# mastbaum/sxmc

Measured on AMD Instinct MI355X. Metric: NLL evals/sec (10^8 samples, 3 obs, 12 signals) + experiments/sec at 1/2/4/8 GPUs, higher is better.
Workload: dtype f64 exact; f32-on-u16-codes filter decides the unambiguous samples

## Files before the change

### sxmc_amd/csrc/nll_device.h

```cpp
#pragma once

#include "sxmc_device.h"

#pragma clang fp contract(off)

namespace sxdev {

constexpr int kWave = 64;

struct Philox4 {
  unsigned x, y, z, w;
};

__device__ __forceinline__ Philox4 philox4x32_10(unsigned long long counter_lo,
                                                 unsigned long long counter_hi,
                                                 unsigned long long key) {
  unsigned c0 = (unsigned)counter_lo, c1 = (unsigned)(counter_lo >> 32);
  unsigned c2 = (unsigned)counter_hi, c3 = (unsigned)(counter_hi >> 32);
  unsigned k0 = (unsigned)key, k1 = (unsigned)(key >> 32);
#pragma unroll
  for (int r = 0; r < 10; r++) {
    const unsigned hi0 = __umulhi(0xD2511F53u, c0), lo0 = 0xD2511F53u * c0;
    const unsigned hi1 = __umulhi(0xCD9E8D57u, c2), lo1 = 0xCD9E8D57u * c2;
    const unsigned n0 = hi1 ^ c1 ^ k0, n1 = lo1, n2 = hi0 ^ c3 ^ k1, n3 = lo0;
    c0 = n0; c1 = n1; c2 = n2; c3 = n3;
    k0 += 0x9E3779B9u;
    k1 += 0xBB67AE85u;
  }
  return Philox4{c0, c1, c2, c3};
}

__device__ __forceinline__ Philox4 rng_next(sxmc_rng_state* st) {
  const Philox4 r = philox4x32_10(st->offset, st->subsequence, st->seed);
  st->offset += 1;
  return r;
}

__device__ __forceinline__ double rng_uniform(sxmc_rng_state* st) {
  const Philox4 r = rng_next(st);
  return ((double)r.x + 1.0) * 2.3283064365386963e-10;
}

__device__ __forceinline__ double rng_normal(sxmc_rng_state* st) {
  const Philox4 r = rng_next(st);
  const double u1 = ((double)r.x + 1.0) * 2.3283064365386963e-10;
  const double u2 = (double)r.y * 2.3283064365386963e-10;
  return sqrt(-2.0 * log(u1)) * cos(6.283185307179586 * u2);
}

__device__ __forceinline__ void pick_new_vector_device(int n, sxmc_rng_state* rng,
                                                       const float* jump_width,
                                                       const double* current_vector,
                                                       double* proposed_vector) {
  const int offset = blockIdx.x * blockDim.x + threadIdx.x;
  const int stride = gridDim.x * blockDim.x;
  for (int i = offset; i < n; i += stride) {
    if (jump_width[i] > 0) {
      const double u = rng_normal(&rng[i]);
      proposed_vector[i] = current_vector[i] + jump_width[i] * u;
    } else {
      proposed_vector[i] = current_vector[i];
    }
  }
}

__device__ __forceinline__ void jump_decider_device(sxmc_rng_state* rng, double* nll_current,
                                                    const double* nll_proposed, double* v_current,
                                                    const double* v_proposed, unsigned nparameters,
                                                    int* accepted, int* counter, float* jump_buffer,
                                                    bool debug_mode) {
  const double u = rng_uniform(&rng[0]);
  const double np = nll_proposed[0];
  const double nc = nll_current[0];
  if (debug_mode || (np < nc || u <= exp(nc - np))) {
    nll_current[0] = np;
    for (unsigned i = 0; i < nparameters; i++) v_current[i] = v_proposed[i];
    accepted[0] += 1;
  }
  const int count = counter[0];
  for (unsigned i = 0; i < nparameters; i++) {
    jump_buffer[count * (nparameters + 1) + i] = (float)v_current[i];
  }
  jump_buffer[count * (nparameters + 1) + nparameters] = (float)nll_current[0];
  counter[0] = count + 1;
}

__device__ __forceinline__ void nll_total_device(size_t nparameters, size_t nsignals, size_t nsources,
                                                 const double* pars, const double* means,
                                                 const double* sigmas, const double* events_total,
                                                 const double* nexpected, const unsigned* n_mc,
                                                 const short* source_id, const unsigned* norms,
                                                 double* nll) {
  double sum = -events_total[0];
  if (isnan(sum)) {
    nll[0] = 1e18;
    return;
  }
  for (unsigned i = 0; i < nsignals; i++) {
    const short sid = source_id[i];
    sum += pars[sid] * nexpected[i] * norms[i] / n_mc[i];
  }
  for (unsigned i = 0; i < nparameters; i++) {
    if (i < nsources && pars[i] < 0) {
      nll[0] = 1e18;
      return;
    }
    if (sigmas[i] > 0) {
      const double x = (pars[i] - means[i]) / sigmas[i];
      sum += 0.5 * x * x;
    }
  }
  nll[0] = sum;
}

template <int BD = 0>
__device__ __forceinline__ double block_sum(size_t n, const double* sums, double* s_wave ) {
  const unsigned bdim = BD > 0 ? (unsigned)BD : blockDim.x;
  double t = 0.0;
  size_t i = threadIdx.x;
  const size_t bd = bdim;
  for (; i + 15 * bd < n; i += 16 * bd) {
    double v[16];
#pragma unroll
    for (int k = 0; k < 16; k++) v[k] = sums[i + (size_t)k * bd];
#pragma unroll
    for (int k = 0; k < 16; k++) t += v[k];
  }
  for (; i < n; i += bd) t += sums[i];
  const int wave = threadIdx.x / kWave;
  const int lane = threadIdx.x & (kWave - 1);
  const int live = min(kWave, (int)bdim - wave * kWave);
#pragma unroll
  for (int off = kWave / 2; off > 0; off >>= 1) {
    const double o = __shfl_down(t, off, kWave);
    t += (lane + off < live) ? o : 0.0;
  }
  const int nwaves = ((int)bdim + kWave - 1) / kWave;
  if ((threadIdx.x & (kWave - 1)) == 0) s_wave[wave] = t;
  __syncthreads();
  if (threadIdx.x == 0) {
    double tot = 0.0;
    for (int w = 0; w < nwaves; w++) tot += s_wave[w];
    s_wave[16] = tot;
  }
  __syncthreads();
  return s_wave[16];
}

constexpr int kStage = 256;

template <int BD = 0, typename Wait>
__device__ __forceinline__ bool finish_step_device_w(size_t npartial_sums, const double* sums, size_t nsignals,
                                                     size_t nsources, const double* means, const double* sigmas,
                                                     sxmc_rng_state* rng, double* nll_current,
                                                     double* nll_proposed, double* v_current, double* v_proposed,
                                                     int* accepted, int* counter, float* jump_buffer,
                                                     int nparameters, const float* jump_width,
                                                     const double* nexpected, const unsigned* n_mc,
                                                     const short* source_id, const unsigned* norms,
                                                     bool debug_mode, Wait&& wait) {
  __shared__ double s_wave[17];
  __shared__ double s_vprop[kStage], s_vcur[kStage], s_pen[kStage], s_z[kStage], s_term[kStage];
  __shared__ float s_jw[kStage];
  __shared__ unsigned char s_flag[kStage];
  __shared__ int s_accept, s_count;
  __shared__ double s_nllcur, s_u;

  const unsigned bdim = BD > 0 ? (unsigned)BD : blockDim.x;
  const bool staged = nparameters <= kStage && nsignals <= (size_t)kStage;
  if (!staged) {
    wait();
    double total_sum = block_sum<BD>(npartial_sums, sums, s_wave);
    if (threadIdx.x == 0) {
      nll_total_device(nparameters, nsignals, nsources, v_proposed, means, sigmas, &total_sum, nexpected, n_mc,
                       source_id, norms, nll_proposed);
      jump_decider_device(rng, nll_current, nll_proposed, v_current, v_proposed, nparameters, accepted, counter,
                          jump_buffer, debug_mode);
    }
    __threadfence_block();
    __syncthreads();
    pick_new_vector_device(nparameters, rng, jump_width, v_current, v_proposed);
    __syncthreads();
    return nll_current[0] == nll_proposed[0];
  }

  double nc = 0.0;
  int count = 0;
  if (threadIdx.x == 0) {
    nc = nll_current[0];
    count = counter[0];
  }
  for (int i = threadIdx.x; i < nparameters; i += (int)bdim) {
    const double p = v_proposed[i], mean = means[i], sigma = sigmas[i];
    const float jw = jump_width[i];
    s_vprop[i] = p;
    s_vcur[i] = v_current[i];
    s_jw[i] = jw;
    unsigned char flag = 0;
    double pen = 0.0;
    if (sigma > 0) {
      const double x = (p - mean) / sigma;
      pen = 0.5 * x * x;
      flag |= 1;
    }
    if ((size_t)i < nsources && p < 0) flag |= 2;
    s_pen[i] = pen;
    s_flag[i] = flag;
    if (i == 0 || jw > 0) {
      sxmc_rng_state st = rng[i];
      if (i == 0) s_u = rng_uniform(&st);
      s_z[i] = (jw > 0) ? rng_normal(&st) : 0.0;
      rng[i].offset = st.offset;
    }
  }
  for (int j = threadIdx.x; j < (int)nsignals; j += (int)bdim) {
    s_term[j] = v_proposed[source_id[j]] * nexpected[j] * norms[j] / n_mc[j];
  }
  wait();
  const double total_sum = block_sum<BD>(npartial_sums, sums, s_wave);

  if (threadIdx.x == 0) {
    double sum = -total_sum;
    bool bad = isnan(sum);
    if (!bad) {
      for (unsigned j = 0; j < nsignals; j++) sum += s_term[j];
      for (int i = 0; i < nparameters; i++) {
        if (s_flag[i] & 2) {
          bad = true;
          break;
        }
        if (s_flag[i] & 1) sum += s_pen[i];
      }
    }
    const double np = bad ? 1e18 : sum;
    nll_proposed[0] = np;
    const bool accept = debug_mode || (np < nc || s_u <= exp(nc - np));
    if (accept) {
      nll_current[0] = np;
      accepted[0] += 1;
    }
    counter[0] = count + 1;
    s_accept = accept ? 1 : 0;
    s_count = count;
    s_nllcur = accept ? np : nc;
  }
  __syncthreads();

  const bool accept = s_accept != 0;
  const size_t row = (size_t)s_count * (size_t)(nparameters + 1);
  for (int i = threadIdx.x; i < nparameters; i += (int)bdim) {
    const double cur = accept ? s_vprop[i] : s_vcur[i];
    if (accept) v_current[i] = cur;
    jump_buffer[row + i] = (float)cur;
    v_proposed[i] = (s_jw[i] > 0) ? cur + s_jw[i] * s_z[i] : cur;
  }
  if (threadIdx.x == 0) jump_buffer[row + nparameters] = (float)s_nllcur;
  return accept;
}

__device__ __forceinline__ bool finish_step_device(size_t npartial_sums, const double* sums, size_t nsignals,
                                                   size_t nsources, const double* means, const double* sigmas,
                                                   sxmc_rng_state* rng, double* nll_current,
                                                   double* nll_proposed, double* v_current, double* v_proposed,
                                                   int* accepted, int* counter, float* jump_buffer,
                                                   int nparameters, const float* jump_width,
                                                   const double* nexpected, const unsigned* n_mc,
                                                   const short* source_id, const unsigned* norms,
                                                   bool debug_mode) {
  return finish_step_device_w<0>(npartial_sums, sums, nsignals, nsources, means, sigmas, rng, nll_current, nll_proposed,
                              v_current, v_proposed, accepted, counter, jump_buffer, nparameters, jump_width, nexpected,
                              n_mc, source_id, norms, debug_mode, [] {});
}

__device__ __forceinline__ void peek_next_proposal_device(int nparameters, const sxmc_rng_state* rng,
                                                          const float* jump_width, const double* v_current,
                                                          double* out) {
  for (int i = threadIdx.x; i < nparameters; i += blockDim.x) {
    const float jw = jump_width[i];
    double v = v_current[i];
    if (jw > 0) {
      sxmc_rng_state st = rng[i];
      if (i == 0) (void)rng_uniform(&st);
      v = v + jw * rng_normal(&st);
    }
    out[i] = v;
  }
}

}
```

### sxmc_amd/csrc/pdfz_kernels.hip

```cpp
#include <hip/hip_runtime.h>
#include <hip/hip_ext.h>

#include <algorithm>
#include <cstring>
#include <vector>

#include "nll_device.h"

#include "fill_kernels.inc.h"

#pragma clang fp contract(off)

namespace {

using namespace sxfill;


__global__ __launch_bounds__(256) void zero_kernel(const SxSignalDesc* __restrict__ descs, unsigned* ticket) {
  const SxSignalDesc& d = descs[blockIdx.y];
  unsigned* bins = d.bins;
  const unsigned n = (unsigned)d.total_nbins;
  const unsigned n4 = n >> 2;
  uint4* b4 = reinterpret_cast<uint4*>(bins);
  const unsigned stride = gridDim.x * blockDim.x;
// ... 147 lines not shown
};
struct MembersFromTable {
  static constexpr bool kTable = true;
  const SxSignalDesc* __restrict__ descs;
  const SxStepEndTable& t;
};

template <int BD = 0, typename Members, typename Ready>
__device__ __forceinline__ double eval_nll_block_part(const Members& mem, int nsig,
                                                      unsigned long long npoints, const unsigned* __restrict__ weight,
                                                      const double* __restrict__ pars,
                                                      const double* __restrict__ nexpected,
                                                      const unsigned* __restrict__ n_mc,
                                                      const short* __restrict__ source_id,
                                                      const unsigned* __restrict__ norms, double* sh,
                                                      unsigned block_index, unsigned nblocks, Ready&& ready) {
  constexpr bool kTable = Members::kTable;
  double* s_wave = sh;
  EvalMember* s_mem = reinterpret_cast<EvalMember*>(sh + 16);
  const unsigned bdim = BD > 0 ? (unsigned)BD : blockDim.x;

  constexpr int U = 16;
  static_assert(!kTable || U == SXMC_STEP_END_MEMBERS, "the table holds one pass of members");
  int rb[U];
  unsigned long long i = (unsigned long long)block_index * bdim + threadIdx.x;
  auto load_read_bins = [&](unsigned long long ev, int j0) {
    const unsigned long long evc = ev < npoints ? ev : npoints - 1;
    gptr<const int> table[U];
#pragma unroll
    for (int u = 0; u < U; u++) {
      if constexpr (kTable) table[u] = to_global(mem.t.read_bins[u]);
      else table[u] = to_global(mem.descs[min(j0 + u, nsig - 1)].read_bins);
    }
#pragma unroll
    for (int u = 0; u < U; u++) rb[u] = table[u][evc];
#pragma unroll
    for (int u = 0; u < U; u++) rb[u] = (j0 + u < nsig && ev < npoints) ? rb[u] : -2;
  };
  auto bins_of = [&](int j0, int u) {
    if constexpr (kTable) return to_global(mem.t.bins[u]);
    else return to_global(s_mem[j0 + u].bins);
  };
  if (npoints == 0 || nsig <= 0) {
    ready();
    return 0.0;
  }
  load_read_bins(i, 0);
  unsigned wfirst = weight ? to_global(weight)[i < npoints ? i : npoints - 1] : 1u;
  unsigned count[U];

  auto stage = [&](int j, const SxSignalDesc& d, unsigned normv, double volume, unsigned nj, unsigned nmc, double par,
                   double nexp) {
    s_mem[j].read_bins = d.read_bins;
    s_mem[j].bins = d.bins;
    s_mem[j].out = d.pdf_out;
    s_mem[j].stride = d.pdf_stride;
    s_mem[j].bin_norm = (double)normv * volume;
    const float eff = (float)(1.0 * nj / nmc);
    s_mem[j].coef = par * nexp * eff;
  };
  if constexpr (kTable) {
    const int j = min((int)threadIdx.x, nsig - 1);
    const SxSignalDesc& d = mem.descs[j];
    const unsigned* normp = d.norm;
    const double volume = d.bin_volume;
    const short sid = source_id[j];
    const unsigned nmc = n_mc[j];
    const double nexp = nexpected[j];
    ready();
    const unsigned nj = norms[j];
    const unsigned normv = *to_global(normp);
    const double par = pars[sid];
#pragma unroll
    for (int u = 0; u < U; u++) count[u] = bins_of(0, u)[rb[u] >= 0 ? rb[u] : 0];
#pragma unroll
    for (int u = 0; u < U; u++) count[u] = (rb[u] >= 0) ? count[u] : 0u;
    stage(j, d, normv, volume, nj, nmc, par, nexp);
  } else {
    ready();
    for (int j = threadIdx.x; j < nsig; j += (int)bdim) {
      const SxSignalDesc& d = mem.descs[j];
      stage(j, d, *to_global((const unsigned*)d.norm), d.bin_volume, norms[j], n_mc[j], pars[source_id[j]], nexpected[j]);
    }
  }
#if SXMC_WG_STAMPS
  if (kTable && BD == 0) {
    asm volatile("s_waitcnt vmcnt(0)" ::: "memory");
    SX_WG_STAMP(1);
  }
#endif
  __syncthreads();

  double sum = 0.0;
  bool requested = true;
  const unsigned long long step = (unsigned long long)nblocks * bdim;
  for (; i < npoints; i += step) {
    double s = 0.0;
    const unsigned wrow = requested ? wfirst : (weight ? to_global(weight)[i] : 1u);
    for (int j0 = 0; j0 < nsig; j0 += U) {
      const bool gathered = kTable && requested;
      if (!requested) load_read_bins(i, j0);
      requested = false;
      if (!gathered) {
#pragma unroll
        for (int u = 0; u < U; u++) count[u] = (rb[u] >= 0) ? bins_of(j0, u)[rb[u]] : 0u;
      }
#if SXMC_WG_STAMPS
      if (!kTable && BD == 0 && i < bdim * nblocks) {
        asm volatile("s_waitcnt vmcnt(0)" ::: "memory");
        SX_WG_STAMP(1);
      }
#endif
#pragma unroll
      for (int u = 0; u < U; u++) {
        if (j0 + u < nsig) {
          float v;
          if (rb[u] == -2) v = 0.0f;
          else if (rb[u] < 0) v = __int_as_float(0x7fc00000);
          else v = (float)((double)count[u] / s_mem[j0 + u].bin_norm);
          if (s_mem[j0 + u].out) to_global(s_mem[j0 + u].out)[s_mem[j0 + u].stride * (long)i] = v;
          s = s + s_mem[j0 + u].coef * (double)(!isnan(v) ? v : 0.0f);
        }
      }
    }
    if (s > 0) sum += weight ? (double)wrow * log(s) : log(s);
  }

#pragma unroll
  for (int off = kWave / 2; off > 0; off >>= 1) sum += __shfl_down(sum, off, kWave);
  const int wave = threadIdx.x / kWave;
  if ((threadIdx.x & (kWave - 1)) == 0) s_wave[wave] = sum;
  __syncthreads();
  double t = 0.0;
  if (threadIdx.x == 0) {
    for (int w = 0; w < (int)(bdim / kWave); w++) t += s_wave[w];
  }
  return t;
}

template <int BD = 0, typename Ready>
__device__ __forceinline__ double eval_nll_block_part(const SxSignalDesc* __restrict__ descs, int nsig,
                                                      unsigned long long npoints, const unsigned* __restrict__ weight,
                                                      const double* __restrict__ pars,
                                                      const double* __restrict__ nexpected,
                                                      const unsigned* __restrict__ n_mc,
                                                      const short* __restrict__ source_id,
                                                      const unsigned* __restrict__ norms, double* sh,
                                                      unsigned block_index, unsigned nblocks, Ready&& ready) {
  return eval_nll_block_part<BD>(MembersFromDescs{descs}, nsig, npoints, weight, pars, nexpected, n_mc, source_id, norms,
                                 sh, block_index, nblocks, ready);
}

template <int BD = 0>
__device__ __forceinline__ double eval_nll_block_part(const SxSignalDesc* __restrict__ descs, int nsig,
                                                      unsigned long long npoints, const unsigned* __restrict__ weight,
                                                      const double* __restrict__ pars,
                                                      const double* __restrict__ nexpected,
                                                      const unsigned* __restrict__ n_mc,
                                                      const short* __restrict__ source_id,
                                                      const unsigned* __restrict__ norms, double* sh,
                                                      unsigned block_index, unsigned nblocks) {
  return eval_nll_block_part<BD>(descs, nsig, npoints, weight, pars, nexpected, n_mc, source_id, norms, sh, block_index,
                                 nblocks, [] {});
}

__device__ __forceinline__ double eval_nll_block(const SxSignalDesc* __restrict__ descs, int nsig,
                                                 unsigned long long npoints, const unsigned* __restrict__ weight,
                                                 const double* __restrict__ pars,
                                                 const double* __restrict__ nexpected,
                                                 const unsigned* __restrict__ n_mc,
                                                 const short* __restrict__ source_id,
                                                 const unsigned* __restrict__ norms, double* sh) {
  return eval_nll_block_part(descs, nsig, npoints, weight, pars, nexpected, n_mc, source_id, norms, sh, blockIdx.x,
                             gridDim.x);
}

__global__ __launch_bounds__(256) void eval_nll_kernel(const SxSignalDesc* __restrict__ descs, int nsig,
                                                       unsigned long long npoints,
                                                       const unsigned* __restrict__ weight,
                                                       const double* __restrict__ pars,
                                                       const double* __restrict__ nexpected,
                                                       const unsigned* __restrict__ n_mc,
                                                       const short* __restrict__ source_id,
                                                       const unsigned* __restrict__ norms,
                                                       double* __restrict__ sums) {
  extern __shared__ double sh[];
  const double t = eval_nll_block(descs, nsig, npoints, weight, pars, nexpected, n_mc, source_id, norms, sh);
  if (threadIdx.x == 0 && !isnan(t)) sums[blockIdx.x] = t;
}

__global__ __launch_bounds__(256) void eval_nll_finish_kernel(const SxSignalDesc* __restrict__ descs, int nsig,
                                                              unsigned long long npoints,
                                                              const unsigned* __restrict__ weight, double* sums,
                                                              unsigned* ticket, SxStepArgs a) {
  extern __shared__ double sh[];
  const double t =
      eval_nll_block(descs, nsig, npoints, weight, a.v_proposed, a.nexpected, a.n_mc, a.source_id, a.norms, sh);
  int* s_last = reinterpret_cast<int*>(sh + 15);
  if (threadIdx.x == 0) {
    sums[blockIdx.x] = isnan(t) ? 0.0 : t;
    asm volatile("s_waitcnt vmcnt(0)" ::: "memory");
    __builtin_amdgcn_fence(__ATOMIC_RELEASE, "agent");
    asm volatile("s_waitcnt vmcnt(0)" ::: "memory");
    const unsigned arrived = __hip_atomic_fetch_add(ticket, 1u, __ATOMIC_RELAXED, __HIP_MEMORY_SCOPE_AGENT);
    const int last = arrived == gridDim.x - 1u;
    if (last) {
      __builtin_amdgcn_fence(__ATOMIC_ACQUIRE, "agent");
      asm volatile("s_waitcnt vmcnt(0)" ::: "memory");
    }
    *s_last = last;
  }
  __syncthreads();
  if (!*s_last) return;
  __syncthreads();
  sxdev::finish_step_device(gridDim.x, sums, a.nsignals, a.nsources, a.means, a.sigmas, a.rng, a.nll_current,
                            a.nll_proposed, a.v_current, a.v_proposed, a.accepted, a.counter, a.jump_buffer,
                            a.nparameters, a.jump_width, a.nexpected, a.n_mc, a.source_id, a.norms,
                            a.debug_mode != 0);
}

__global__ __launch_bounds__(256) void eval_nll2_kernel(const SxSignalDesc* __restrict__ descs_a,
                                                        const SxSignalDesc* __restrict__ descs_b, int nsig,
                                                        unsigned long long npoints,
                                                        const unsigned* __restrict__ weight_a,
                                                        const unsigned* __restrict__ weight_b,
                                                        const double* __restrict__ pars_a,
                                                        const double* __restrict__ pars_b,
                                                        const double* __restrict__ nexpected,
                                                        const unsigned* __restrict__ n_mc,
                                                        const short* __restrict__ source_id,
                                                        const unsigned* __restrict__ norms_a,
                                                        const unsigned* __restrict__ norms_b,
                                                        double* __restrict__ sums_a, double* __restrict__ sums_b,
                                                        unsigned half) {
  extern __shared__ double sh[];
  const bool second = blockIdx.x >= half;
  const double t = eval_nll_block_part(second ? descs_b : descs_a, nsig, npoints, second ? weight_b : weight_a,
                                       second ? pars_b : pars_a, nexpected, n_mc, source_id,
                                       second ? norms_b : norms_a, sh, second ? blockIdx.x - half : blockIdx.x, half);
  if (threadIdx.x == 0 && !isnan(t)) (second ? sums_b : sums_a)[second ? blockIdx.x - half : blockIdx.x] = t;
}

__global__ __launch_bounds__(256) void finish2_zero_kernel(const SxSignalDesc* __restrict__ descs_a,
                                                           const SxSignalDesc* __restrict__ descs_b, int nsig,
                                                           unsigned zblocks, size_t npartial, const double* sums_a,
                                                           const double* sums_b, const unsigned* norms_b, double* v_b,
                                                           const int* cap, SxStepArgs a) {
  if (blockIdx.x == 0) {
    __shared__ int s_before;
    if (threadIdx.x == 0) s_before = a.counter[0];
    __syncthreads();
    const int limit = cap ? cap[0] : 0x7FFFFFFF;
    if (s_before < limit) {
      const bool accepted =
          sxdev::finish_step_device(npartial, sums_a, a.nsignals, a.nsources, a.means, a.sigmas, a.rng, a.nll_current,
                                    a.nll_proposed, a.v_current, a.v_proposed, a.accepted, a.counter, a.jump_buffer,
                                    a.nparameters, a.jump_width, a.nexpected, a.n_mc, a.source_id, a.norms,
                                    a.debug_mode != 0);
      __syncthreads();
      if (!accepted && s_before + 1 < limit) {
        sxdev::finish_step_device(npartial, sums_b, a.nsignals, a.nsources, a.means, a.sigmas, a.rng, a.nll_current,
                                  a.nll_proposed, a.v_current, a.v_proposed, a.accepted, a.counter, a.jump_buffer,
                                  a.nparameters, a.jump_width, a.nexpected, a.n_mc, a.source_id, norms_b,
                                  a.debug_mode != 0);
        __syncthreads();
      }
      sxdev::peek_next_proposal_device(a.nparameters, a.rng, a.jump_width, a.v_current, v_b);
    }
    __syncthreads();
    for (int j = threadIdx.x; j < nsig; j += blockDim.x) {
      *descs_a[j].norm = 0u;
      *descs_b[j].norm = 0u;
    }
    return;
  }
  const unsigned b = blockIdx.x - 1u;
  const unsigned which = b / (zblocks * (unsigned)nsig);
  const unsigned bb = b - which * zblocks * (unsigned)nsig;
  const SxSignalDesc& d = (which ? descs_b : descs_a)[bb / zblocks];
  const unsigned chunk = bb % zblocks;
  unsigned* bins = d.bins;
  const unsigned n = (unsigned)d.total_nbins;
  const unsigned n4 = n >> 2;
  uint4* b4 = reinterpret_cast<uint4*>(bins);
  const unsigned stride = zblocks * blockDim.x;
  for (unsigned i = chunk * blockDim.x + threadIdx.x; i < n4; i += stride) b4[i] = make_uint4(0u, 0u, 0u, 0u);
  if (chunk == 0 && threadIdx.x < (n & 3u)) bins[(n4 << 2) + threadIdx.x] = 0u;
}

__global__ void peek_next_proposal_kernel(int nparameters, const sxmc_rng_state* rng, const float* jump_width,
                                          const double* v_current, double* out) {
  sxdev::peek_next_proposal_device(nparameters, rng, jump_width, v_current, out);
}

__global__ __launch_bounds__(1024) void tail_step_kernel(const SxSignalDesc* __restrict__ descs, int nsig,
                                                         unsigned long long npoints,
                                                         const unsigned* __restrict__ weight, SxStepArgs a) {
  extern __shared__ double sh[];
  __shared__ double s_total;
  const double t =
      eval_nll_block(descs, nsig, npoints, weight, a.v_proposed, a.nexpected, a.n_mc, a.source_id, a.norms, sh);
  if (threadIdx.x == 0) s_total = isnan(t) ? 0.0 : t;
  __syncthreads();
  sxdev::finish_step_device(1, &s_total, a.nsignals, a.nsources, a.means, a.sigmas, a.rng, a.nll_current,
                            a.nll_proposed, a.v_current, a.v_proposed, a.accepted, a.counter, a.jump_buffer,
                            a.nparameters, a.jump_width, a.nexpected, a.n_mc, a.source_id, a.norms,
                            a.debug_mode != 0);
  for (int j = 0; j < nsig; j++) {
    const SxSignalDesc& d = descs[j];
    const unsigned n = (unsigned)d.total_nbins, n4 = n >> 2;
    uint4* b4 = reinterpret_cast<uint4*>(d.bins);
    for (unsigned i = threadIdx.x; i < n4; i += blockDim.x) b4[i] = make_uint4(0u, 0u, 0u, 0u);
    if (threadIdx.x < (n & 3u)) d.bins[(n4 << 2) + threadIdx.x] = 0u;
    if (threadIdx.x == 0) *d.norm = 0u;
  }
}

__global__ __launch_bounds__(256) void finish_zero_kernel(const SxSignalDesc* __restrict__ descs, int nsig,
                                                          unsigned zblocks, size_t npartial, const double* sums,
                                                          unsigned* ticket, SxStepArgs a) {
  if (blockIdx.x == 0) {
    sxdev::finish_step_device(npartial, sums, a.nsignals, a.nsources, a.means, a.sigmas, a.rng, a.nll_current,
                              a.nll_proposed, a.v_current, a.v_proposed, a.accepted, a.counter, a.jump_buffer,
                              a.nparameters, a.jump_width, a.nexpected, a.n_mc, a.source_id, a.norms,
                              a.debug_mode != 0);
    __syncthreads();
    for (int j = threadIdx.x; j < nsig; j += blockDim.x) *descs[j].norm = 0u;
    if (threadIdx.x == 0 && ticket) *ticket = 0u;
    return;
  }
  const unsigned b = blockIdx.x - 1u;
  const SxSignalDesc& d = descs[b / zblocks];
  const unsigned chunk = b % zblocks;
  unsigned* bins = d.bins;
  const unsigned n = (unsigned)d.total_nbins;
  const unsigned n4 = n >> 2;
  uint4* b4 = reinterpret_cast<uint4*>(bins);
  const unsigned stride = zblocks * blockDim.x;
  for (unsigned i = chunk * blockDim.x + threadIdx.x; i < n4; i += stride) b4[i] = make_uint4(0u, 0u, 0u, 0u);
  if (chunk == 0 && threadIdx.x < (n & 3u)) bins[(n4 << 2) + threadIdx.x] = 0u;
}

constexpr unsigned kEndSpinLimit = 200000u;
constexpr unsigned long long kSlotEmpty = 0x7FF8DEADBEEF0001ull, kSlotNaN = 0x7FF8DEADBEEF0002ull;

template <int BD, typename Members, typename Ready>
__device__ __forceinline__ void step_end_role(unsigned role, unsigned W, const Members& lookup,
                                              const SxSignalDesc* __restrict__ hist_descs, int nsig,
                                              unsigned long long npoints, const unsigned* __restrict__ weight,
                                              unsigned long long* slots, double* last_good, unsigned* sync,
                                              unsigned nvb, unsigned zblocks, const SxStepArgs& a, double* sh,
                                              Ready&& ready) {
  const unsigned bdim = BD > 0 ? (unsigned)BD : blockDim.x;
  unsigned* const timeouts = sync + 6;
  if (role == W) {
    ready();
    __shared__ double s_part[128];
    sxdev::finish_step_device_w<BD>(nvb, s_part, a.nsignals, a.nsources, a.means, a.sigmas, a.rng, a.nll_current,
                                    a.nll_proposed, a.v_current, a.v_proposed, a.accepted, a.counter, a.jump_buffer,
                                    a.nparameters, a.jump_width, a.nexpected, a.n_mc, a.source_id, a.norms,
                                    a.debug_mode != 0, [&] {
                                      const unsigned i = threadIdx.x;
                                      if (i < nvb) {
                                        unsigned long long v = kSlotEmpty;
                                        unsigned it = 0;
                                        for (; it < kEndSpinLimit; it++) {
                                          v = __hip_atomic_load(slots + i, __ATOMIC_RELAXED, __HIP_MEMORY_SCOPE_AGENT);
                                          if (v != kSlotEmpty) break;
                                          __builtin_amdgcn_s_sleep(1);
                                        }
                                        double t;
                                        if (v == kSlotEmpty) {
                                          __hip_atomic_fetch_add(timeouts, 1u, __ATOMIC_RELAXED, __HIP_MEMORY_SCOPE_AGENT);
                                          t = 0.0;
                                        } else if (v == kSlotNaN) {
                                          t = last_good[i];
                                        } else {
                                          t = __longlong_as_double((long long)v);
                                          last_good[i] = t;
                                        }
                                        s_part[i] = t;
                                      }
                                      __syncthreads();
                                      if (BD == 0) SX_WG_STAMP(1);
                                      if (i < nvb) {
                                        __hip_atomic_store(slots + i, kSlotEmpty, __ATOMIC_RELAXED, __HIP_MEMORY_SCOPE_AGENT);
                                      }
                                    });
    __syncthreads();
#if SXMC_MEASURE
    if (a.gate && threadIdx.x == 0) {
      __threadfence();
      __hip_atomic_store(a.gate, a.gate_value, __ATOMIC_RELAXED, __HIP_MEMORY_SCOPE_AGENT);
    }
#endif
    for (int j = threadIdx.x; j < nsig; j += (int)bdim) *hist_descs[j].norm = 0u;
    if (threadIdx.x == 0) sync[0] = 0u;
    if (BD == 0) SX_WG_STAMP(2);
    return;
  }
  const unsigned vb = role;
  const double t = eval_nll_block_part<BD>(lookup, nsig, npoints, weight, a.v_proposed, a.nexpected, a.n_mc,
                                           a.source_id, a.norms, sh, vb, nvb, ready);
  __shared__ int s_clear;
  if (threadIdx.x == 0) {
    __hip_atomic_store(slots + vb, isnan(t) ? kSlotNaN : (unsigned long long)__double_as_longlong(t), __ATOMIC_RELAXED,
                       __HIP_MEMORY_SCOPE_AGENT);
    asm volatile("s_waitcnt vmcnt(0)" ::: "memory");
    if (BD == 0) SX_WG_STAMP(2);
    unsigned it = 0;
    for (; it < kEndSpinLimit; it++) {
      if (__hip_atomic_load(slots + vb, __ATOMIC_RELAXED, __HIP_MEMORY_SCOPE_AGENT) == kSlotEmpty) break;
      __builtin_amdgcn_s_sleep(1);
    }
    if (it == kEndSpinLimit) __hip_atomic_fetch_add(timeouts, 1u, __ATOMIC_RELAXED, __HIP_MEMORY_SCOPE_AGENT);
    s_clear = it < kEndSpinLimit ? 1 : 0;
  }
  __syncthreads();
  if (!s_clear) return;
  const unsigned npieces = zblocks * (unsigned)nsig;
  for (unsigned p = role; p < npieces; p += W) {
    const SxSignalDesc& d = hist_descs[p / zblocks];
    const unsigned chunk = p % zblocks;
    unsigned* bins = d.bins;
    const unsigned n = (unsigned)d.total_nbins;
    const unsigned n4 = n >> 2;
    uint4* b4 = reinterpret_cast<uint4*>(bins);
    const unsigned stride = zblocks * bdim;
    for (unsigned i = chunk * bdim + threadIdx.x; i < n4; i += stride) b4[i] = make_uint4(0u, 0u, 0u, 0u);
    if (chunk == 0 && threadIdx.x < (n & 3u)) bins[(n4 << 2) + threadIdx.x] = 0u;
  }
}

template <bool TABLE>
__global__ __launch_bounds__(128) void step_end_kernel(const SxSignalDesc* __restrict__ lookup_descs,
                                                       const SxSignalDesc* __restrict__ hist_descs, int nsig,
                                                       unsigned long long npoints, const unsigned* __restrict__ weight,
                                                       unsigned long long* slots, double* last_good, unsigned* sync,
                                                       unsigned nvb, unsigned zblocks, SxStepArgs a, SxStepEndTable table) {
  extern __shared__ double sh[];
  SX_WG_STAMP(0);
  if constexpr (TABLE) {
    step_end_role<0>(blockIdx.x, gridDim.x - 1u, MembersFromTable{lookup_descs, table}, hist_descs, nsig, npoints, weight, slots,
                     last_good, sync, nvb, zblocks, a, sh, [] {});
  } else {
    step_end_role<0>(blockIdx.x, gridDim.x - 1u, MembersFromDescs{lookup_descs}, hist_descs, nsig, npoints, weight, slots,
                     last_good, sync, nvb, zblocks, a, sh, [] {});
  }
}

struct SxTailArgs {
  const SxSignalDesc* lookup_descs;
  const SxSignalDesc* hist_descs;
  int nsig;
  unsigned nvb, zblocks, pad;
  unsigned long long npoints;
  const unsigned* weight;
  unsigned long long* slots;
  double* last_good;
  unsigned* sync;
  SxStepArgs a;
};

template <typename Fill>
__device__ __forceinline__ void fill_step_body(unsigned nfill, const SxTailArgs& t, unsigned dbg, Fill&& fill) {
  if (blockIdx.x < nfill) {
    fill();
    asm volatile("s_waitcnt vmcnt(0)" ::: "memory");
    __syncthreads();
    if (threadIdx.x == 0) __hip_atomic_fetch_add(t.sync + 7, 1u, __ATOMIC_RELAXED, __HIP_MEMORY_SCOPE_AGENT);
    return;
  }
  if (threadIdx.x >= 128u) return;
  if (sxfill::sx_dbg(dbg) & 8u) return;
  SX_WG_STAMP(0);
  extern __shared__ double sh_tail[];
  const unsigned role_index = blockIdx.x - nfill;
  const unsigned W = t.nvb;
  const unsigned role = role_index == 0 ? W : role_index - 1u;
  auto fill_done = [&] {
    if (threadIdx.x == 0) {
      unsigned* done = t.sync + 7;
      unsigned it = 0;
      for (; it < kEndSpinLimit; it++) {
        if (__hip_atomic_load(done, __ATOMIC_RELAXED, __HIP_MEMORY_SCOPE_AGENT) >= nfill) break;
        __builtin_amdgcn_s_sleep(1);
      }
      if (it == kEndSpinLimit) __hip_atomic_fetch_add(t.sync + 6, 1u, __ATOMIC_RELAXED, __HIP_MEMORY_SCOPE_AGENT);
    }
    SX_WG_STAMP(1);
    __syncthreads();
  };
  step_end_role<128>(role, W, MembersFromDescs{t.lookup_descs}, t.hist_descs, t.nsig, t.npoints, t.weight, t.slots, t.last_good, t.sync,
                     t.nvb, t.zblocks, t.a, sh_tail, fill_done);
  if (role == W && threadIdx.x == 0) {
    __hip_atomic_store(t.sync + 7, 0u, __ATOMIC_RELAXED, __HIP_MEMORY_SCOPE_AGENT);
  }
  SX_WG_STAMP(2);
}

template <int NOBS, int NSLOT, typename PROG>
__global__ __launch_bounds__(1024) void fill_ordered_step_kernel(const SxSignalDesc* __restrict__ descs,
                                                                 const SxSegment* __restrict__ segs,
                                                                 const unsigned* __restrict__ blk_off, unsigned layout,
                                                                 unsigned dbg, unsigned nfill, SxTailArgs tail) {
  fill_step_body(nfill, tail, dbg, [&] {
    SxChainDescs one;
    one.d[0] = one.d[1] = one.d[2] = one.d[3] = descs;
    fill_ordered_body<NOBS, NSLOT, PROG, 1, true>(one, segs, blk_off, layout, dbg);
  });
}

template <int NOBS, int NSLOT, typename PROG, int PREW>
__global__ __launch_bounds__(1024) void fill_step_kernel(const SxSignalDesc* __restrict__ descs,
                                                         const SxSegment* __restrict__ segs,
                                                         const unsigned* __restrict__ blk_off, unsigned hist_words,
                                                         unsigned dbg, unsigned nfill, SxTailArgs tail) {
  fill_step_body(nfill, tail, dbg, [&] { fill_body<NOBS, NSLOT, true, PROG, PREW>(descs, segs, blk_off, hist_words, dbg); });
}

__global__ __launch_bounds__(128) void step_end2_kernel(const SxSignalDesc* __restrict__ lookup_a,
                                                        const SxSignalDesc* __restrict__ lookup_b,
                                                        const SxSignalDesc* __restrict__ hist_a,
                                                        const SxSignalDesc* __restrict__ hist_b, int nsig,
                                                        unsigned long long npoints, const unsigned* __restrict__ weight_a,
                                                        const unsigned* __restrict__ weight_b, unsigned long long* slots,
                                                        double* last_good, unsigned* sync, unsigned nvb, unsigned zblocks,
                                                        const unsigned* norms_b, double* v_b, const int* cap, SxStepArgs a) {
  extern __shared__ double sh[];
  const unsigned W = gridDim.x - 1u;
  unsigned* const timeouts = sync + 6;
  if (blockIdx.x == W) {
    __shared__ double s_part[128];
    __shared__ int s_before;
    if (threadIdx.x == 0) s_before = a.counter[0];
    __syncthreads();
    const int limit = cap ? cap[0] : 0x7FFFFFFF;
    auto collect = [&] {
      const unsigned i = threadIdx.x;
      if (i < W) {
        unsigned long long v = kSlotEmpty;
        for (unsigned it = 0; it < kEndSpinLimit; it++) {
          v = __hip_atomic_load(slots + i, __ATOMIC_RELAXED, __HIP_MEMORY_SCOPE_AGENT);
          if (v != kSlotEmpty) break;
          __builtin_amdgcn_s_sleep(1);
        }
        double t;
        if (v == kSlotEmpty) {
          __hip_atomic_fetch_add(timeouts, 1u, __ATOMIC_RELAXED, __HIP_MEMORY_SCOPE_AGENT);
          t = 0.0;
        } else if (v == kSlotNaN) {
          t = last_good[i];
        } else {
          t = __longlong_as_double((long long)v);
          last_good[i] = t;
        }
        s_part[i] = t;
      }
      __syncthreads();
      if (i < W) __hip_atomic_store(slots + i, kSlotEmpty, __ATOMIC_RELAXED, __HIP_MEMORY_SCOPE_AGENT);
    };
    if (s_before < limit) {
      const bool accepted = sxdev::finish_step_device_w(
          nvb, s_part, a.nsignals, a.nsources, a.means, a.sigmas, a.rng, a.nll_current, a.nll_proposed, a.v_current,
          a.v_proposed, a.accepted, a.counter, a.jump_buffer, a.nparameters, a.jump_width, a.nexpected, a.n_mc,
          a.source_id, a.norms, a.debug_mode != 0, collect);
      __syncthreads();
      if (!accepted && s_before + 1 < limit) {
        sxdev::finish_step_device(nvb, s_part + nvb, a.nsignals, a.nsources, a.means, a.sigmas, a.rng, a.nll_current,
                                  a.nll_proposed, a.v_current, a.v_proposed, a.accepted, a.counter, a.jump_buffer,
                                  a.nparameters, a.jump_width, a.nexpected, a.n_mc, a.source_id, norms_b,
                                  a.debug_mode != 0);
        __syncthreads();
      }
      sxdev::peek_next_proposal_device(a.nparameters, a.rng, a.jump_width, a.v_current, v_b);
    } else {
      collect();
    }
    __syncthreads();
    for (int j = threadIdx.x; j < nsig; j += blockDim.x) {
      *hist_a[j].norm = 0u;
      *hist_b[j].norm = 0u;
    }
    return;
  }
  const bool second = blockIdx.x >= nvb;
  const unsigned vb = second ? blockIdx.x - nvb : blockIdx.x;
  const double t = eval_nll_block_part(second ? lookup_b : lookup_a, nsig, npoints, second ? weight_b : weight_a,
                                       second ? v_b : a.v_proposed, a.nexpected, a.n_mc, a.source_id,
                                       second ? norms_b : a.norms, sh, vb, nvb);
  __shared__ int s_clear;
  if (threadIdx.x == 0) {
    __hip_atomic_store(slots + blockIdx.x, isnan(t) ? kSlotNaN : (unsigned long long)__double_as_longlong(t),
                       __ATOMIC_RELAXED, __HIP_MEMORY_SCOPE_AGENT);
    asm volatile("s_waitcnt vmcnt(0)" ::: "memory");
    unsigned it = 0;
    for (; it < kEndSpinLimit; it++) {
      if (__hip_atomic_load(slots + blockIdx.x, __ATOMIC_RELAXED, __HIP_MEMORY_SCOPE_AGENT) == kSlotEmpty) break;
      __builtin_amdgcn_s_sleep(1);
    }
    if (it == kEndSpinLimit) __hip_atomic_fetch_add(timeouts, 1u, __ATOMIC_RELAXED, __HIP_MEMORY_SCOPE_AGENT);
    s_clear = it < kEndSpinLimit ? 1 : 0;
  }
  __syncthreads();
  if (!s_clear) return;
  const unsigned npieces = 2u * zblocks * (unsigned)nsig;
  for (unsigned p = blockIdx.x; p < npieces; p += W) {
    const unsigned which = p / (zblocks * (unsigned)nsig);
    const unsigned q = p - which * zblocks * (unsigned)nsig;
    const SxSignalDesc& d = (which ? hist_b : hist_a)[q / zblocks];
    const unsigned chunk = q % zblocks;
    unsigned* bins = d.bins;
    const unsigned n = (unsigned)d.total_nbins;
    const unsigned n4 = n >> 2;
    uint4* b4 = reinterpret_cast<uint4*>(bins);
    const unsigned stride = zblocks * blockDim.x;
    for (unsigned i = chunk * blockDim.x + threadIdx.x; i < n4; i += stride) b4[i] = make_uint4(0u, 0u, 0u, 0u);
    if (chunk == 0 && threadIdx.x < (n & 3u)) bins[(n4 << 2) + threadIdx.x] = 0u;
  }
}

__global__ __launch_bounds__(256) void eval_nll_chains_kernel(SxChainEnds e, int nsig) {
  extern __shared__ double sh[];
  const SxChainEnd& c = e.c[blockIdx.y];
  if (blockIdx.x >= c.nblocks) return;
  const double t = eval_nll_block_part(c.lookup_descs, nsig, c.nrows, c.weight, c.a.v_proposed, c.a.nexpected, c.a.n_mc,
                                       c.a.source_id, c.a.norms, sh, blockIdx.x, c.nblocks);
  if (threadIdx.x == 0 && !isnan(t)) c.sums[blockIdx.x] = t;
}

__global__ __launch_bounds__(256) void finish_zero_chains_kernel(SxChainEnds e, int nsig, unsigned zblocks) {
  const SxChainEnd& c = e.c[blockIdx.y];
  const SxStepArgs& a = c.a;
  if (blockIdx.x == 0) {
    sxdev::finish_step_device(c.nblocks, c.sums, a.nsignals, a.nsources, a.means, a.sigmas, a.rng, a.nll_current,
                              a.nll_proposed, a.v_current, a.v_proposed, a.accepted, a.counter, a.jump_buffer,
                              a.nparameters, a.jump_width, a.nexpected, a.n_mc, a.source_id, a.norms,
                              a.debug_mode != 0);
    __syncthreads();
    for (int j = threadIdx.x; j < nsig; j += blockDim.x) *c.hist_descs[j].norm = 0u;
    if (threadIdx.x == 0 && c.ticket) *c.ticket = 0u;
    return;
  }
  const unsigned b = blockIdx.x - 1u;
  const SxSignalDesc& d = c.hist_descs[b / zblocks];
  const unsigned chunk = b % zblocks;
  unsigned* bins = d.bins;
  const unsigned n = (unsigned)d.total_nbins;
  const unsigned n4 = n >> 2;
  uint4* b4 = reinterpret_cast<uint4*>(bins);
  const unsigned stride = zblocks * blockDim.x;
  for (unsigned i = chunk * blockDim.x + threadIdx.x; i < n4; i += stride) b4[i] = make_uint4(0u, 0u, 0u, 0u);
  if (chunk == 0 && threadIdx.x < (n & 3u)) bins[(n4 << 2) + threadIdx.x] = 0u;
}

#if SXMC_WG_STAMPS
extern "C" {
__device__ unsigned long long sx_wg_stamps[3 * 4096];
}
extern "C" int sxmc_debug_read_wg_stamps(unsigned long long* out, int n) {
  return (int)hipMemcpyFromSymbol(out, HIP_SYMBOL(sx_wg_stamps), sizeof(unsigned long long) * (size_t)n);
}
#endif

__global__ __launch_bounds__(256) void prebin_kernel(const SxSignalDesc* __restrict__ dp, unsigned mask, int width,
                                                     void* out) {
  const SxSignalDesc& d = *dp;
  const unsigned long long npad = d.nvec * SXMC_VEC;
  const unsigned sentinel = width == 1 ? 0xFFu : width == 2 ? 0xFFFFu : 0xFFFFFFFFu;
  const unsigned long long step = (unsigned long long)gridDim.x * blockDim.x;
  for (unsigned long long i = (unsigned long long)blockIdx.x * blockDim.x + threadIdx.x; i < npad; i += step) {
    unsigned val = sentinel;
    if (i < d.nsamples) {
      bool ok = true;
      int part = 0;
      for (int k = 0; k < d.nobs; k++) {
        if (!((mask >> k) & 1u)) continue;
        const double x = (double)to_global(d.cols)[(unsigned long long)k * d.col_pitch + i];
        ok = ok && (x >= d.lower[k]) && (x < d.upper[k]);
        part += (int)((x - d.lower[k]) * d.scale[k]) * d.bin_stride[k];
      }
      if (ok) val = (unsigned)part;
    }
    if (width == 1) static_cast<unsigned char*>(out)[i] = (unsigned char)val;
    else if (width == 2) static_cast<unsigned short*>(out)[i] = (unsigned short)val;
    else static_cast<unsigned*>(out)[i] = val;
  }
}

#if SXMC_MEASURE
__global__ void pow_int_kernel(const double* __restrict__ x, int n, int i, double* __restrict__ out) {
  for (int k = blockIdx.x * blockDim.x + threadIdx.x; k < n; k += gridDim.x * blockDim.x) {
    double h = 1.0, l = 0.0;
    for (int t = 0; t < i; t++) pow_step(h, l, x[k]);
    out[k] = h;
  }
}
#endif

__global__ __launch_bounds__(256) void transpose_kernel(const float* __restrict__ aos, float* __restrict__ cols,
                                                        unsigned long long n, int F,
                                                        unsigned long long pitch) {
  const unsigned long long npad = (n + SXMC_VEC - 1) / SXMC_VEC * SXMC_VEC;
  const unsigned long long step = (unsigned long long)gridDim.x * blockDim.x;
  for (unsigned long long i = (unsigned long long)blockIdx.x * blockDim.x + threadIdx.x; i < npad; i += step) {
    for (int k = 0; k < F; k++) {
      cols[(unsigned long long)k * pitch + i] = (i < n) ? aos[i * F + k] : __int_as_float(0x7fc00000);
    }
  }
}

__global__ __launch_bounds__(256) void untranspose_obs_kernel(const float* __restrict__ cols, float* __restrict__ out,
                                                              unsigned long long n, int nobs,
                                                              unsigned long long pitch, float dataset) {
  const unsigned long long step = (unsigned long long)gridDim.x * blockDim.x;
  for (unsigned long long i = (unsigned long long)blockIdx.x * blockDim.x + threadIdx.x; i < n; i += step) {
    for (int k = 0; k < nobs; k++) out[i * (nobs + 1) + k] = cols[(unsigned long long)k * pitch + i];
    out[i * (nobs + 1) + nobs] = dataset;
  }
}

template <typename K, typename... A>
hipError_t launch_fill(const SxLaunchShape& sh, K k, size_t lds, bool fused, hipStream_t s, A... args) {
  if (lds > 48 * 1024) {
    hipError_t e = hipFuncSetAttribute(reinterpret_cast<const void*>(k), hipFuncAttributeMaxDynamicSharedMemorySize,
                                       (int)lds);
    if (e != hipSuccess) return e;
  }
// ... 389 lines not shown
```

Measured before the change: 13330.

## Parallelize MCMC step finish: all threads compute decision, drop serial loops and barrier

Every thread in the finish step now preloads the signal and penalty terms into registers and takes the accept/reject decision itself. A wave ballot replaces the per-parameter flag scan, which removes the thread-0 serial summation and the trailing barrier. The end-step kernel also moves the histogram norm clears into the wait callback and caches the histogram bin ranges in shared memory before spinning, so the zeroing pass reads less global descriptor data. The trade-off is more register pressure from the unrolled add array. Summation order also changes (penalties now add -0.0 instead of being skipped), and the shared-memory HistRange overlay relies on the member-record layout.

```diff
diff --git a/sxmc_amd/csrc/nll_device.h b/sxmc_amd/csrc/nll_device.h
--- a/sxmc_amd/csrc/nll_device.h
+++ b/sxmc_amd/csrc/nll_device.h
@@ -149,7 +149,7 @@
 
 constexpr int kStage = 256;
 
-template <int BD = 0, typename Wait>
+template <int BD = 0, int R = (BD > 0 ? 8 : 32), typename Wait>
 __device__ __forceinline__ bool finish_step_device_w(size_t npartial_sums, const double* sums, size_t nsignals,
                                                      size_t nsources, const double* means, const double* sigmas,
                                                      sxmc_rng_state* rng, double* nll_current,
@@ -160,11 +160,12 @@
                                                      const short* source_id, const unsigned* norms,
                                                      bool debug_mode, Wait&& wait) {
   __shared__ double s_wave[17];
-  __shared__ double s_vprop[kStage], s_vcur[kStage], s_pen[kStage], s_z[kStage], s_term[kStage];
+  __shared__ double s_vprop[kStage], s_vcur[kStage], s_z[kStage];
+  __shared__ double s_add[2 * kStage];
   __shared__ float s_jw[kStage];
-  __shared__ unsigned char s_flag[kStage];
-  __shared__ int s_accept, s_count;
-  __shared__ double s_nllcur, s_u;
+  __shared__ unsigned s_badw[16];
+  __shared__ int s_count, s_nacc;
+  __shared__ double s_nc, s_u;
 
   const unsigned bdim = BD > 0 ? (unsigned)BD : blockDim.x;
   const bool staged = nparameters <= kStage && nsignals <= (size_t)kStage;
@@ -179,33 +180,38 @@
     }
     __threadfence_block();
     __syncthreads();
-    pick_new_vector_device(nparameters, rng, jump_width, v_current, v_proposed);
+    for (int i = threadIdx.x; i < nparameters; i += (int)bdim) {
+      if (jump_width[i] > 0) {
+        const double u = rng_normal(&rng[i]);
+        v_proposed[i] = v_current[i] + jump_width[i] * u;
+      } else {
+        v_proposed[i] = v_current[i];
+      }
+    }
     __syncthreads();
     return nll_current[0] == nll_proposed[0];
   }
 
-  double nc = 0.0;
-  int count = 0;
   if (threadIdx.x == 0) {
-    nc = nll_current[0];
-    count = counter[0];
-  }
+    s_nc = nll_current[0];
+    s_count = counter[0];
+    s_nacc = accepted[0];
+  }
+  double* const s_pen = s_add + nsignals;
+  bool negative_rate = false;
   for (int i = threadIdx.x; i < nparameters; i += (int)bdim) {
     const double p = v_proposed[i], mean = means[i], sigma = sigmas[i];
     const float jw = jump_width[i];
     s_vprop[i] = p;
     s_vcur[i] = v_current[i];
     s_jw[i] = jw;
-    unsigned char flag = 0;
-    double pen = 0.0;
+    double pen = -0.0;
     if (sigma > 0) {
       const double x = (p - mean) / sigma;
       pen = 0.5 * x * x;
-      flag |= 1;
-    }
-    if ((size_t)i < nsources && p < 0) flag |= 2;
+    }
+    if ((size_t)i < nsources && p < 0) negative_rate = true;
     s_pen[i] = pen;
-    s_flag[i] = flag;
     if (i == 0 || jw > 0) {
       sxmc_rng_state st = rng[i];
       if (i == 0) s_u = rng_uniform(&st);
@@ -214,50 +220,63 @@
     }
   }
   for (int j = threadIdx.x; j < (int)nsignals; j += (int)bdim) {
-    s_term[j] = v_proposed[source_id[j]] * nexpected[j] * norms[j] / n_mc[j];
-  }
+    s_add[j] = v_proposed[source_id[j]] * nexpected[j] * norms[j] / n_mc[j];
+  }
+  const int nwaves = ((int)bdim + kWave - 1) / kWave;
+  {
+    const unsigned long long any_negative = __ballot(negative_rate);
+    if ((threadIdx.x & (kWave - 1)) == 0) s_badw[threadIdx.x / kWave] = any_negative != 0ull ? 1u : 0u;
+  }
+  __syncthreads();
+  constexpr int kRegAdd = R;
+  static_assert(R > 0 && R % 8 == 0, "whole blocks of eight additions");
+  const int nadd = (int)nsignals + nparameters;
+  double add[kRegAdd];
+#pragma unroll
+  for (int k = 0; k < kRegAdd; k++) add[k] = s_add[min(k, max(nadd - 1, 0))];
+#pragma unroll
+  for (int k = 0; k < kRegAdd; k++) add[k] = k < nadd ? add[k] : -0.0;
+  bool bad = false;
+  for (int w = 0; w < nwaves; w++) bad = bad || s_badw[w] != 0u;
+  const double nc = s_nc, u = s_u;
+  const int count = s_count, nacc = s_nacc;
   wait();
   const double total_sum = block_sum<BD>(npartial_sums, sums, s_wave);
 
+  double sum = -total_sum;
+  bad = bad || isnan(sum);
+#pragma unroll
+  for (int k0 = 0; k0 < kRegAdd; k0 += 8) {
+    if (k0 < nadd) {
+#pragma unroll
+      for (int k = 0; k < 8; k++) sum += add[k0 + k];
+    }
+  }
+  for (int k = kRegAdd; k < nadd; k++) sum += s_add[k];
+  const double np = bad ? 1e18 : sum;
+  const bool accept = debug_mode || (np < nc || u <= exp(nc - np));
   if (threadIdx.x == 0) {
-    double sum = -total_sum;
-    bool bad = isnan(sum);
-    if (!bad) {
-      for (unsigned j = 0; j < nsignals; j++) sum += s_term[j];
-      for (int i = 0; i < nparameters; i++) {
-        if (s_flag[i] & 2) {
-          bad = true;
-          break;
-        }
-        if (s_flag[i] & 1) sum += s_pen[i];
-      }
-    }
-    const double np = bad ? 1e18 : sum;
     nll_proposed[0] = np;
-    const bool accept = debug_mode || (np < nc || s_u <= exp(nc - np));
     if (accept) {
       nll_current[0] = np;
-      accepted[0] += 1;
+      accepted[0] = nacc + 1;
     }
     counter[0] = count + 1;
-    s_accept = accept ? 1 : 0;
-    s_count = count;
-    s_nllcur = accept ? np : nc;
-  }
-  __syncthreads();
-
-  const bool accept = s_accept != 0;
-  const size_t row = (size_t)s_count * (size_t)(nparameters + 1);
+  }
+
+  const double nllcur = accept ? np : nc;
+  const size_t row = (size_t)count * (size_t)(nparameters + 1);
   for (int i = threadIdx.x; i < nparameters; i += (int)bdim) {
     const double cur = accept ? s_vprop[i] : s_vcur[i];
     if (accept) v_current[i] = cur;
     jump_buffer[row + i] = (float)cur;
     v_proposed[i] = (s_jw[i] > 0) ? cur + s_jw[i] * s_z[i] : cur;
   }
-  if (threadIdx.x == 0) jump_buffer[row + nparameters] = (float)s_nllcur;
+  if (threadIdx.x == 0) jump_buffer[row + nparameters] = (float)nllcur;
   return accept;
 }
 
+template <int R = 32>
 __device__ __forceinline__ bool finish_step_device(size_t npartial_sums, const double* sums, size_t nsignals,
                                                    size_t nsources, const double* means, const double* sigmas,
                                                    sxmc_rng_state* rng, double* nll_current,
@@ -267,7 +286,7 @@
                                                    const double* nexpected, const unsigned* n_mc,
                                                    const short* source_id, const unsigned* norms,
                                                    bool debug_mode) {
-  return finish_step_device_w<0>(npartial_sums, sums, nsignals, nsources, means, sigmas, rng, nll_current, nll_proposed,
+  return finish_step_device_w<0, R>(npartial_sums, sums, nsignals, nsources, means, sigmas, rng, nll_current, nll_proposed,
                               v_current, v_proposed, accepted, counter, jump_buffer, nparameters, jump_width, nexpected,
                               n_mc, source_id, norms, debug_mode, [] {});
 }
diff --git a/sxmc_amd/csrc/pdfz_kernels.hip b/sxmc_amd/csrc/pdfz_kernels.hip
--- a/sxmc_amd/csrc/pdfz_kernels.hip
+++ b/sxmc_amd/csrc/pdfz_kernels.hip
@@ -473,7 +473,7 @@
       eval_nll_block(descs, nsig, npoints, weight, a.v_proposed, a.nexpected, a.n_mc, a.source_id, a.norms, sh);
   if (threadIdx.x == 0) s_total = isnan(t) ? 0.0 : t;
   __syncthreads();
-  sxdev::finish_step_device(1, &s_total, a.nsignals, a.nsources, a.means, a.sigmas, a.rng, a.nll_current,
+  sxdev::finish_step_device<8>(1, &s_total, a.nsignals, a.nsources, a.means, a.sigmas, a.rng, a.nll_current,
                             a.nll_proposed, a.v_current, a.v_proposed, a.accepted, a.counter, a.jump_buffer,
                             a.nparameters, a.jump_width, a.nexpected, a.n_mc, a.source_id, a.norms,
                             a.debug_mode != 0);
@@ -527,6 +527,8 @@
   if (role == W) {
     ready();
     __shared__ double s_part[128];
+    unsigned* const my_norm = nsig > 0 ? hist_descs[min((int)threadIdx.x, nsig - 1)].norm : nullptr;
+    const bool clear_in_wait = a.nparameters <= sxdev::kStage && a.nsignals <= (size_t)sxdev::kStage;
     sxdev::finish_step_device_w<BD>(nvb, s_part, a.nsignals, a.nsources, a.means, a.sigmas, a.rng, a.nll_current,
                                     a.nll_proposed, a.v_current, a.v_proposed, a.accepted, a.counter, a.jump_buffer,
                                     a.nparameters, a.jump_width, a.nexpected, a.n_mc, a.source_id, a.norms,
@@ -557,6 +559,7 @@
                                       if (i < nvb) {
                                         __hip_atomic_store(slots + i, kSlotEmpty, __ATOMIC_RELAXED, __HIP_MEMORY_SCOPE_AGENT);
                                       }
+                                      if (clear_in_wait && (int)i < nsig) *my_norm = 0u;
                                     });
     __syncthreads();
 #if SXMC_MEASURE
@@ -565,7 +568,8 @@
       __hip_atomic_store(a.gate, a.gate_value, __ATOMIC_RELAXED, __HIP_MEMORY_SCOPE_AGENT);
     }
 #endif
-    for (int j = threadIdx.x; j < nsig; j += (int)bdim) *hist_descs[j].norm = 0u;
+    if (!clear_in_wait && (int)threadIdx.x < nsig) *my_norm = 0u;
+    for (int j = (int)(threadIdx.x + bdim); j < nsig; j += (int)bdim) *hist_descs[j].norm = 0u;
     if (threadIdx.x == 0) sync[0] = 0u;
     if (BD == 0) SX_WG_STAMP(2);
     return;
@@ -577,6 +581,18 @@
   if (threadIdx.x == 0) {
     __hip_atomic_store(slots + vb, isnan(t) ? kSlotNaN : (unsigned long long)__double_as_longlong(t), __ATOMIC_RELAXED,
                        __HIP_MEMORY_SCOPE_AGENT);
+  }
+  struct HistRange {
+    unsigned* bins;
+    unsigned n, pad;
+  };
+  static_assert(sizeof(HistRange) <= sizeof(EvalMember), "parked over the member records");
+  HistRange* const s_hist = reinterpret_cast<HistRange*>(sh + 16);
+  for (int j = threadIdx.x; j < nsig; j += (int)bdim) {
+    s_hist[j].bins = hist_descs[j].bins;
+    s_hist[j].n = (unsigned)hist_descs[j].total_nbins;
+  }
+  if (threadIdx.x == 0) {
     asm volatile("s_waitcnt vmcnt(0)" ::: "memory");
     if (BD == 0) SX_WG_STAMP(2);
     unsigned it = 0;
@@ -591,10 +607,10 @@
   if (!s_clear) return;
   const unsigned npieces = zblocks * (unsigned)nsig;
   for (unsigned p = role; p < npieces; p += W) {
-    const SxSignalDesc& d = hist_descs[p / zblocks];
+    const HistRange d = s_hist[p / zblocks];
     const unsigned chunk = p % zblocks;
     unsigned* bins = d.bins;
-    const unsigned n = (unsigned)d.total_nbins;
+    const unsigned n = d.n;
     const unsigned n4 = n >> 2;
     uint4* b4 = reinterpret_cast<uint4*>(bins);
     const unsigned stride = zblocks * bdim;
```

Result: faster. 13860 (median of 6 runs) (+4.0%).
